# mapbox/robosat

Hardware: AMD Instinct MI355X
Metric: 512x512 tiles/sec train+predict, 1/2/4/8 MI355X; mIoU vs CPU ref (higher is better)
Workload: dtype f32; 1 GPU; rs predict ResNet50-UNet, bs=16 3x512x512 fp32 per GPU, 2 classes (BASELINE configs[1]); parallelism=tiles sharded over 1 rank(s), no collective

## Files before the change

include/robosat_hip.h:

```cpp
#ifndef ROBOSAT_HIP_H
#define ROBOSAT_HIP_H

#include <stdint.h>

#ifdef __cplusplus
extern "C" {
#endif

#define RS_EINVAL (-22)

typedef void* rs_stream_t;

typedef uint16_t rs_bf16;
#define RS_F32 0
#define RS_BF16 1

int rs_abi_version(void);

typedef struct rs_conv_desc {
  int32_t N;
  int32_t Hs, Ws;
  int32_t C1, C2;
  int32_t ups;
  int32_t kh, kw, stride, pad;
  int32_t Ho, Wo;
  int32_t Cout;
  int32_t relu;
  int32_t stem;
} rs_conv_desc;

int rs_conv2d_fwd(const rs_conv_desc* d, const float* src1, const float* src2, const float* weight,
                  const float* scale, const float* shift, const float* residual, const float* relu_mask, float* out,
                  rs_stream_t stream);

int rs_conv2d_tile(const rs_conv_desc* d);
const char* rs_conv2d_tile_name(int tile);

int rs_pack_stem_weight(const float* w_krsc, float* packed, int Cout, int kh, int kw, int Cin, rs_stream_t stream);


int rs_nchw_to_nhwc4(const float* x, float* y, int N, int C, int H, int W, rs_stream_t stream);

int rs_maxpool2d_fwd(const float* x, float* y, uint8_t* argmax, int N, int H, int W, int C, int k, int stride, int pad,
                     int Ho, int Wo, rs_stream_t stream);

int rs_bn_fold(const float* gamma, const float* beta, const float* mean, const float* var, float eps, float* scale,
               float* shift, int C, rs_stream_t stream);

int rs_final_conv1x1(const float* x, const float* w, const float* bias, float* out, int N, int H, int W, int Cin,
                     int C, int softmax, rs_stream_t stream);



long rs_conv2d_wgrad_workspace_bytes(const rs_conv_desc* d);
int rs_conv2d_wgrad_form(const rs_conv_desc* d);
int rs_conv2d_wgrad(const rs_conv_desc* d, const float* dy, const float* src1, const float* src2, float* dw,
                    void* workspace, rs_stream_t stream);
int rs_unpack_stem_weight(const float* packed, float* w_krsc, int Cout, int kh, int kw, int Cin, rs_stream_t stream);

int rs_pack_dgrad_weight(const float* w_krsc, float* out, int Cout, int kh, int kw, int Cin, rs_stream_t stream);

long rs_bn_workspace_bytes(long M, int C);
int rs_bn_train_stats(const float* y, long M, int C, float eps, float momentum, const float* gamma, const float* beta,
                      float* mean, float* invstd, float* scale, float* shift, float* running_mean, float* running_var,
                      long long* num_batches_tracked, void* workspace, rs_stream_t stream);
int rs_bn_apply(const float* y, const float* scale, const float* shift, const float* residual, float* out, long M, int C,
                int relu, rs_stream_t stream);
int rs_bn_bwd(const float* dz, const float* zmask, const float* y, const float* mean, const float* invstd,
              const float* gamma, float* dy, float* dmasked, float* dgamma, float* dbeta, long M, int C, void* workspace,
              rs_stream_t stream);

// ... 232 lines not shown
```

robosat_amd/_lib.py:

```python

import ctypes
import os
from ctypes import POINTER, c_char_p, c_float, c_int, c_int32, c_long, c_void_p

import torch

_HERE = os.path.dirname(os.path.abspath(__file__))
LIB_PATH = os.environ.get("ROBOSAT_HIP_LIB") or os.path.join(_HERE, "librobosat_hip.so")

RS_EINVAL = -22
ABI_VERSION = 24
RS_F32, RS_BF16 = 0, 1
RS_TTA_IN_U8, RS_TTA_IN_F32 = 0, 1
RS_TTA_PROBS, RS_TTA_QUANTIZE, RS_TTA_ARGMAX = 0, 1, 2


class ConvDesc(ctypes.Structure):

    _fields_ = [
        ("N", c_int32), ("Hs", c_int32), ("Ws", c_int32), ("C1", c_int32), ("C2", c_int32), ("ups", c_int32),
        ("kh", c_int32), ("kw", c_int32), ("stride", c_int32), ("pad", c_int32), ("Ho", c_int32), ("Wo", c_int32),
        ("Cout", c_int32), ("relu", c_int32), ("stem", c_int32),
    ]


P = c_void_p

SIGNATURES = {
    "rs_abi_version": (c_int, []),
    "rs_conv2d_fwd": (c_int, [POINTER(ConvDesc), P, P, P, P, P, P, P, P, P]),
    "rs_conv2d_tile": (c_int, [POINTER(ConvDesc)]),
    "rs_conv2d_tile_name": (c_char_p, [c_int]),
    "rs_pack_stem_weight": (c_int, [P, P, c_int, c_int, c_int, c_int, P]),
    "rs_nchw_to_nhwc4": (c_int, [P, P, c_int, c_int, c_int, c_int, P]),
    "rs_maxpool2d_fwd": (c_int, [P, P, P, c_int, c_int, c_int, c_int, c_int, c_int, c_int, c_int, c_int, P]),
    "rs_bn_fold": (c_int, [P, P, P, P, c_float, P, P, c_int, P]),
    "rs_final_conv1x1": (c_int, [P, P, P, P, c_int, c_int, c_int, c_int, c_int, c_int, P]),
    "rs_conv2d_wgrad_workspace_bytes": (c_long, [POINTER(ConvDesc)]),
    "rs_conv2d_wgrad": (c_int, [POINTER(ConvDesc), P, P, P, P, P, P]),
    "rs_unpack_stem_weight": (c_int, [P, P, c_int, c_int, c_int, c_int, P]),
    "rs_pack_dgrad_weight": (c_int, [P, P, c_int, c_int, c_int, c_int, P]),
    "rs_bn_workspace_bytes": (c_long, [c_long, c_int]),
    "rs_bn_train_stats": (c_int, [P, c_long, c_int, c_float, c_float, P, P, P, P, P, P, P, P, P, P, P]),
    "rs_bn_apply": (c_int, [P, P, P, P, P, c_long, c_int, c_int, P]),
    "rs_bn_bwd": (c_int, [P, P, P, P, P, P, P, P, P, P, c_long, c_int, P, P]),
    "rs_maxpool2d_bwd": (c_int, [P, P, P, c_int, c_int, c_int, c_int, c_int, c_int, c_int, c_int, c_int, c_int, P]),
    "rs_upsample2x_bwd": (c_int, [P, P, P, P, P, c_int, c_int, c_int, c_int, c_int, c_int, P]),
    "rs_final_conv1x1_bwd_workspace_bytes": (c_long, [c_int, c_int]),
    "rs_final_conv1x1_bwd": (c_int, [P, P, P, P, P, P, c_int, c_int, c_int, c_int, c_int, c_int, P, P]),
    "rs_nll_loss_workspace_bytes": (c_long, []),
    "rs_nll_loss_fwd": (c_int, [P, P, P, P, P, c_int, c_int, c_int, c_int, c_int, c_float, P, P]),
    "rs_nll_loss_bwd": (c_int, [P, P, P, P, P, P, c_int, c_int, c_int, c_int, c_int, c_float, P]),
    "rs_miou_loss_workspace_bytes": (c_long, [c_int, c_int]),
    "rs_miou_loss_fwd": (c_int, [P, P, P, P, P, c_int, c_int, c_int, c_int, P, P]),
    "rs_miou_loss_bwd": (c_int, [P, P, P, P, P, P, c_int, c_int, c_int, c_int, P]),
    "rs_lovasz_workspace_bytes": (c_long, [c_int, c_int, c_int, c_int]),
    "rs_lovasz_fwd": (c_int, [P, P, P, P, c_int, c_int, c_int, c_int, P, P]),
    "rs_scale_by_scalar": (c_int, [P, P, P, c_long, P]),
    "rs_lovasz_softmax_workspace_bytes": (c_long, [c_int, c_int, c_int, c_int, c_int]),
    "rs_lovasz_softmax_fwd": (c_int, [P, P, P, P, P, c_int, c_int, c_int, c_int, c_int, c_int, P, P]),
    "rs_confusion_counts": (c_int, [P, P, P, c_int, c_int, c_int, c_int, P]),
    "rs_conv2d_fwd_bf16": (c_int, [POINTER(ConvDesc), P, P, P, P, P, P, P, P, P]),
    "rs_conv2d_tile_bf16": (c_int, [POINTER(ConvDesc)]),
    "rs_conv2d_config": (c_int, [POINTER(ConvDesc), c_int, c_int, POINTER(c_int), POINTER(c_int)]),
    "rs_conv2d_set_tuning": (c_int, [c_int, c_int]),
    "rs_set_knob": (c_int, [c_char_p, c_int]),
# ... 131 lines not shown
```

robosat_amd/autograd.py:

```python

import torch

from . import ops


_SIDE = {}


def _side_stream(device):

    if torch.device(device).type != "cuda":
        return None
    if not ops.switch("ROBOSAT_WGRAD_STREAM"):
        return torch.cuda.current_stream(device)
    s = _SIDE.get(device)
    if s is None:
        s = torch.cuda.Stream(device=device)
        _SIDE[device] = s
    return s


class GradArena:

    TRACE = None
# ... 135 lines not shown
    ready.record(main)
    side.wait_event(ready)
    with torch.cuda.stream(side):
        packed = []
        for blk in (net.center, net.dec0, net.dec1, net.dec2, net.dec3, net.dec4):
            conv = blk.block.block
            packed += [conv.phase(dt), conv.dgrad_phase(dt)]
            if dt == torch.float32 and getattr(conv, "_phase_wino", None) is not None:
                packed.append(conv.phase_wino())
            if dt == torch.float32 and getattr(conv, "_dgrad_phase_wino", None) is not None:
                packed.append(conv.dgrad_phase_wino())
    done = torch.cuda.Event()
    done.record(side)
    for w in packed:
        w.record_stream(main)
    return done


def _forward(net, x, tape, backward=False):
    from .unet import _bump_generation

    _bump_generation()
    decoder_weights_ready = _prefetch_decoder_weights(net, net.compute_dtype, x.device)
    r = net.resnet
    t = tape.t
    dt = net.compute_dtype
    if dt == torch.bfloat16:
        net.prep_bf16_weights()
    elif backward:
        net.prep_f32_weights()
    x4 = ops.nchw_to_nhwc4(x, dt)
    t["x4"] = x4
    if dt == torch.bfloat16:
        y0 = ops.stem_conv_bf16(x4, ops.pack_stem_weight(r.conv1.krsc(), dt))
    else:
        y0 = ops.conv2d(x4, ops.pack_stem_weight(r.conv1.krsc()), stride=2, pad=3, stem=7, bands=net.in_channels)
    z0, st0 = _bn_train(r.bn1, y0)
    p0, am0 = ops.maxpool2d(z0, 3, 2, 1, want_argmax=True)
    t.update(y0=y0, st0=st0, z0=z0, am0=am0)

    h = p0
    enc = []
    for layer in net._blocks():
        for blk in layer:
            rec = {"blk": blk, "h": h}
            y1, z1, rec["st1"], rec["b1"] = _conv_bn(blk.bn1, h, blk.conv1.krsc(dt))
            y2, z2, rec["st2"], rec["b2"] = _conv_bn(blk.bn2, z1, blk.conv2.krsc(dt), stride=blk.stride, pad=1, conv=blk.conv2)
            if blk.downsample is not None:
                yd, idt, rec["std"], _ = _conv_bn(blk.downsample[1], h, blk.downsample[0].krsc(dt), stride=blk.stride, relu=False)
                rec["yd"] = yd
            else:
                idt = h
            y3, z3, rec["st3"], rec["b3"] = _conv_bn(blk.bn3, z2, blk.conv3.krsc(dt), residual=idt, relu=True)
            rec.update(y1=y1, z1=z1, y2=y2, z2=z2, y3=y3, z3=z3)
            tape.blocks.append(rec)
            h = z3
        enc.append(h)
    enc1, enc2, enc3, enc4 = enc

    def up(block, skip, prev=None):
        from .unet import decoder_block

        return decoder_block(block.block.block, skip, prev, dt)

    pooled, amc = ops.maxpool2d(enc4, 2, 2, 0, want_argmax=True)
    if decoder_weights_ready is not None:
        torch.cuda.current_stream(x.device).wait_event(decoder_weights_ready)
    center = up(net.center, pooled)
    dec0 = up(net.dec0, enc4, center)
# ... 198 lines not shown
```

robosat_amd/csrc/common.h:

```cpp
#pragma once
#include <hip/hip_runtime.h>
#include <stdint.h>

#include "../../include/robosat_hip.h"

typedef float f32x4 __attribute__((ext_vector_type(4)));
typedef float f32x16 __attribute__((ext_vector_type(16)));
typedef __bf16 bf16_t;
typedef __bf16 bf16x4 __attribute__((ext_vector_type(4)));
typedef __bf16 bf16x8 __attribute__((ext_vector_type(8)));
typedef unsigned int u32x2 __attribute__((ext_vector_type(2)));
typedef unsigned int u32x4 __attribute__((ext_vector_type(4)));
typedef short s16x4 __attribute__((ext_vector_type(4)));
typedef short s16x8 __attribute__((ext_vector_type(8)));

__device__ __forceinline__ f32x4 rs_ld4(const float* p) { return *reinterpret_cast<const f32x4*>(p); }
__device__ __forceinline__ f32x4 rs_ld4(const bf16_t* p) {
  return __builtin_convertvector(*reinterpret_cast<const bf16x4*>(p), f32x4);
}
__device__ __forceinline__ void rs_st4(float* p, f32x4 v) { *reinterpret_cast<f32x4*>(p) = v; }
__device__ __forceinline__ void rs_st4(bf16_t* p, f32x4 v) {
  *reinterpret_cast<bf16x4*>(p) = __builtin_convertvector(v, bf16x4);
}
__device__ __forceinline__ float rs_ld1(const float* p) { return *p; }
// ... 130 lines not shown
struct rs_fastdiv {
  unsigned int mul;
  unsigned int shift;
  unsigned int div;
};

static inline rs_fastdiv rs_make_fastdiv(unsigned int d) {
  rs_fastdiv f;
  unsigned int s = 0;
  while ((1ull << s) < d) ++s;
  f.shift = s;
  f.mul = (unsigned int)((((1ull << s) - d) << 32) / d + 1);
  f.div = d;
  return f;
}

__host__ __device__ __forceinline__ unsigned int rs_div(unsigned int n, const rs_fastdiv f) {
#if defined(__HIP_DEVICE_COMPILE__)
  return (__umulhi(n, f.mul) + n) >> f.shift;
#else
  return (unsigned int)((((unsigned long long)n * f.mul) >> 32) + n) >> f.shift;
#endif
}

struct RsKnobs {
  int conv_tile = -1;
  int conv_rowb = 0;
  int conv_big = 1;
  int conv_min256 = 384;
  int conv_halo = 1;
  int conv_halo_min = 192;
  int conv_halo512 = -1;
  int conv_splitk = -1;
  int conv1x1_ew = -1;
  int conv1x1_np = 0;
  int conv1x1_ew_bf16 = 0;
  int halo_ko = 0;
  int wgrad_f32_phase = 1;
  int wgrad_f32_dma = -1;
  int wgrad_f32_blocks = 2048;
  int wgrad_f32_wino = 1;
  int wgrad_f32_wino_blocks = 1024;
  int wgrad_f32_wino33 = 1;
  int wgrad_f32_wino33_blocks = 256;
  int wgrad_blocks = 96;
  int wgrad_blocks_phase = 1536;
  int wgrad_phase4 = 1;
  int wgrad_blocks_phase4 = 256;
  int wgrad_ring = 3;
  int lovasz_xcd = 1;
  int wino_wide = 1;
};
__attribute__((visibility("hidden"))) RsKnobs& rs_knobs();

__attribute__((visibility("hidden"))) int rs_wgrad_thin_plan(const rs_conv_desc* d, int* blocks, int* slices);
__attribute__((visibility("hidden"))) int rs_wgrad_thin_launch(const rs_conv_desc* d, const void* dy, const void* src,
                                                               float* partial, void* stream);

__attribute__((visibility("hidden"))) int rs_conv_thin_bf16_launch(int mode, const void* src, const void* wgt, const void* mask,
                                                                   void* out, int N, int Hs, int Ws, int relu, void* stream);

__attribute__((visibility("hidden"))) long rs_reduce_scratch_floats(long n, int splits);
__attribute__((visibility("hidden"))) int rs_reduce_splits(const float* ws, float* out, long n, int splits, float* scratch,
                                                           void* stream);

__attribute__((visibility("hidden"))) int rs_conv_dma_f32(const rs_conv_desc* d, const float* src1, const float* src2,
// ... 5 lines not shown
```

robosat_amd/csrc/knobs.hip:

```cpp
#include <stdio.h>
#include <stdlib.h>
#include <string.h>

#include "common.h"

namespace {

struct Entry {
  const char* name;
  const char* env;
  int RsKnobs::*field;
  int lo, hi;
};

bool in_range(const Entry& e, int v) {
  if (v < e.lo || v > e.hi) return false;
  if (e.field == &RsKnobs::conv_rowb) return v == 0 || v == 64 || v == 128;
  return true;
}

const Entry kEntries[] = {
    {"conv_tile", "RS_CONV_TILE", &RsKnobs::conv_tile, -1, 9},
    {"conv_rowb", "RS_CONV_ROWB", &RsKnobs::conv_rowb, 0, 128},
    {"conv_big", "RS_CONV_BIG", &RsKnobs::conv_big, 0, 1},
    {"conv_min256", "RS_CONV_MIN256", &RsKnobs::conv_min256, 0, 1048576},
    {"conv_halo", "RS_CONV_HALO", &RsKnobs::conv_halo, 0, 1},
    {"conv_halo_min", "RS_CONV_HALO_MIN", &RsKnobs::conv_halo_min, 0, 1048576},
    {"conv_halo512", "RS_CONV_HALO512", &RsKnobs::conv_halo512, -1, 1},
    {"conv_splitk", "RS_CONV_SPLITK", &RsKnobs::conv_splitk, -1, 16},
    {"conv1x1_ew", "RS_CONV1X1_EW", &RsKnobs::conv1x1_ew, -1, 1},
    {"conv1x1_np", "RS_CONV1X1_NP", &RsKnobs::conv1x1_np, -1, 1},
    {"conv1x1_ew_bf16", "RS_CONV1X1_EW_BF16", &RsKnobs::conv1x1_ew_bf16, 0, 1},
    {"halo_ko", "RS_HALO_KO", &RsKnobs::halo_ko, 0, 4},
    {"wgrad_f32_phase", "RS_WGRAD_F32_PHASE", &RsKnobs::wgrad_f32_phase, 0, 1},
    {"wgrad_f32_dma", "RS_WGRAD_F32_DMA", &RsKnobs::wgrad_f32_dma, -1, 1},
    {"wgrad_f32_blocks", "RS_WGRAD_F32_BLOCKS", &RsKnobs::wgrad_f32_blocks, 1, 1048576},
    {"wgrad_f32_wino", "RS_WGRAD_F32_WINO", &RsKnobs::wgrad_f32_wino, 0, 1},
    {"wgrad_f32_wino_blocks", "RS_WGRAD_F32_WINO_BLOCKS", &RsKnobs::wgrad_f32_wino_blocks, 1, 1048576},
    {"wgrad_f32_wino33", "RS_WGRAD_F32_WINO33", &RsKnobs::wgrad_f32_wino33, 0, 1},
    {"wgrad_f32_wino33_blocks", "RS_WGRAD_F32_WINO33_BLOCKS", &RsKnobs::wgrad_f32_wino33_blocks, 1, 1048576},
    {"wgrad_blocks", "RS_WGRAD_BLOCKS", &RsKnobs::wgrad_blocks, 1, 1048576},
    {"wgrad_blocks_phase", "RS_WGRAD_BLOCKS_PHASE", &RsKnobs::wgrad_blocks_phase, 1, 1048576},
    {"wgrad_phase4", "RS_WGRAD_PHASE4", &RsKnobs::wgrad_phase4, 0, 1},
    {"wgrad_blocks_phase4", "RS_WGRAD_BLOCKS_PHASE4", &RsKnobs::wgrad_blocks_phase4, 1, 1048576},
    {"wgrad_ring", "RS_WGRAD_RING", &RsKnobs::wgrad_ring, 2, 7},
    {"lovasz_xcd", "RS_LOVASZ_XCD", &RsKnobs::lovasz_xcd, 0, 1},
    {"wino_wide", "ROBOSAT_WINO_WIDE", &RsKnobs::wino_wide, 0, 1},
};

}

RsKnobs& rs_knobs() {
  static RsKnobs k = [] {
    RsKnobs v;
    for (const Entry& e : kEntries)
      if (const char* s = getenv(e.env)) {
        const int x = atoi(s);
        if (in_range(e, x)) v.*(e.field) = x;
        else fprintf(stderr, "robosat_hip: %s=%s is outside [%d, %d]: ignored, the rule stays\n", e.env, s, e.lo, e.hi);
      }
    return v;
  }();
// ... 24 lines not shown
```

robosat_amd/csrc/stem_f32.hip:

```cpp
#include "lds_dma.h"

namespace {

struct StemArgs {
  const float* x;
  const float* w;
  const float* scale;
  const float* shift;
  float* out;
  int N, H, W, Ho, Wo, relu;
  int tpr;
  int ntile;
#ifdef RS_STEM_TRACE
  long long* trace;
#endif
};

constexpr int SBM = 128, SBN = 64;
constexpr int SCOLS = 2 * SBM + 6;
constexpr int XI = 132;
constexpr int LDO = SBN + 4;

template <int CIN>
struct Geom {
  static constexpr int PS = CIN == 3 ? 3 : 5;
  static constexpr int ROWF = 2 * XI * PS;
  static constexpr int STRIPF = 7 * ROWF;
  static constexpr int PAIR = 7 * CIN;
  static constexpr int NPAIR = 3 * PAIR;
  static constexpr int NEO = 3 * CIN;
  static constexpr int NSTEP = NPAIR + NEO + CIN;
  static constexpr int WF = NSTEP * 2 * SBN;
  static constexpr int STAGEF = SBM * LDO;
  static constexpr int REGION = STRIPF > STAGEF ? STRIPF : STAGEF;
  static constexpr int ZEROF = SBM * PS + 8;
  static constexpr int LDSF = WF + REGION + ZEROF;
};

struct Tap {
  int r, s, c;
};
template <int CIN>
__host__ __device__ constexpr Tap stem_tap(int t, int h) {
  using G = Geom<CIN>;
  if (t < G::NPAIR) return Tap{2 * (t / G::PAIR) + h, (t % G::PAIR) / CIN, t % CIN};
  const int u = t - G::NPAIR;
  return Tap{6, 2 * (u / CIN) + h, u % CIN};
}
template <int CIN>
__host__ __device__ constexpr int stem_imm(int t) {
  using G = Geom<CIN>;
  const Tap k = stem_tap<CIN>(t, 0);
  return ((k.r * 2 + (k.s & 1)) * XI + (k.s >> 1)) * G::PS + k.c;
}

template <int CIN>
__global__ __launch_bounds__(256, CIN == 3 ? 2 : 1) void stem_conv_f32(const StemArgs p) {
  using G = Geom<CIN>;
  constexpr int PS = G::PS;
  constexpr int NPF = (7 * SCOLS + 255) / 256;
  static_assert(G::LDSF * 4 <= (CIN == 3 ? 80 : 160) * 1024, "LDS");

  __shared__ __attribute__((aligned(16))) float lds[G::LDSF];
  float* const wl = lds;
  float* const strip = lds + G::WF;
  float* const zline = lds + G::WF + G::REGION;

  const int tid = threadIdx.x;
  const int lane = tid & 63;
  const int wave = tid >> 6;
  const int wm = wave >> 1, wn = wave & 1;
  const int li = lane & 31, lh = lane >> 5;

#ifdef RS_STEM_TRACE
  if (tid == 0) p.trace[((long)blockIdx.x * 64 + 63) * 8 + 0] = (long long)__builtin_amdgcn_s_memtime();
#endif
  const int t0 = (int)((long)blockIdx.x * p.ntile / gridDim.x);
  const int t1 = (int)((long)(blockIdx.x + 1) * p.ntile / gridDim.x);
  if (t0 >= t1) return;

  {
    constexpr int NW4 = SBN * 7 * 8 / 256;
    f32x4 wv[NW4];
#pragma unroll
    for (int k = 0; k < NW4; ++k) wv[k] = *reinterpret_cast<const f32x4*>(p.w + (tid + 256 * k) * 4);
#pragma unroll
    for (int k = 0; k < NW4; ++k) {
      const int e = tid + 256 * k;
      const int s_ = e & 7, r = (e >> 3) % 7, co = e / 56;
      int t, h;
      if (r < 6) {
        t = (r >> 1) * G::PAIR + s_ * CIN, h = r & 1;
        if (s_ == 7) continue;
      } else if (s_ < 6) {
        t = G::NPAIR + (s_ >> 1) * CIN, h = s_ & 1;
      } else {
        t = G::NPAIR + G::NEO, h = s_ & 1;
      }
#pragma unroll
      for (int c = 0; c < CIN; ++c) wl[((t + c) * 2 + h) * SBN + co] = wv[k][c];
    }
  }
  for (int e = tid; e < G::ZEROF; e += 256) zline[e] = 0.f;

  f32x4 pf[NPF];
  int pdst[NPF];
  int prow[NPF], pcol[NPF], prel[NPF];
#pragma unroll
  for (int q = 0; q < NPF; ++q) {
    const int e = tid + 256 * q;
    const int r = e / SCOLS, j = e - r * SCOLS;
    const bool in = e < 7 * SCOLS;
    pdst[q] = in ? ((r * 2 + (j & 1)) * XI + (j >> 1)) * PS : -1;
    prow[q] = in ? r : -(1 << 24);
    pcol[q] = j;
    prel[q] = (r * p.W + j) * 16;
  }
  const long img = (long)p.H * p.W * 4;
  int cn, coy, ctx;
  {
    const int rowt = t0 / p.tpr;
    ctx = t0 - rowt * p.tpr;
    cn = rowt / p.Ho;
    coy = rowt - cn * p.Ho;
  }
  auto fetch = [&](int n, int oy, int tx, bool live) __attribute__((always_inline)) {
    const __amdgpu_buffer_rsrc_t rs = rs_dma_rsrc<0x7FFFFFF0u>(p.x + n * img, live ? img * 4 : 0);
    const int iy0 = 2 * oy - 3, ix0 = 2 * tx * SBM - 3;
    const int base = (iy0 * p.W + ix0) * 16;
#pragma unroll
    for (int q = 0; q < NPF; ++q) {
      const bool ok = (unsigned)(iy0 + prow[q]) < (unsigned)p.H && (unsigned)(ix0 + pcol[q]) < (unsigned)p.W;
      pf[q] = __builtin_bit_cast(f32x4, __builtin_amdgcn_raw_buffer_load_b128(rs, ok ? base + prel[q] : -1, 0, 0));
    }
  };
  auto put = [&]() __attribute__((always_inline)) {
#pragma unroll
    for (int q = 0; q < NPF; ++q) {
      if (pdst[q] >= 0) {
        float* d = strip + pdst[q];
        d[0] = pf[q][0];
        d[1] = pf[q][1];
        d[2] = pf[q][2];
        if (CIN == 4) d[3] = pf[q][3];
      }
    }
  };

  const int apix = (wm * 64 + li) * PS;
  const float* const A1 = strip + apix + lh * G::ROWF;
  const float* const A2 = strip + apix + lh * (XI * PS);
  constexpr int IMM6 = ((6 * 2 + 0) * XI + 3) * PS;
  const float* const A3 = lh ? zline + apix - IMM6 : strip + apix;
  const float* const B = wl + lh * SBN + wn * 32 + li;

  const int ecol = (tid & 15) * 4, erow = tid >> 4;
  f32x4 sc = {1.f, 1.f, 1.f, 1.f}, sh = {0.f, 0.f, 0.f, 0.f};
  if (p.scale) sc = *reinterpret_cast<const f32x4*>(p.scale + ecol);
  if (p.shift) sh = *reinterpret_cast<const f32x4*>(p.shift + ecol);

#ifdef RS_STEM_TRACE
#define STAMP(k) do { if (tid == 0) p.trace[((long)blockIdx.x * 64 + (tile - t0)) * 8 + (k)] = (long long)__builtin_amdgcn_s_memtime(); } while (0)
#else
#define STAMP(k)
#endif
#ifdef RS_STEM_TRACE
  if (tid == 0) p.trace[((long)blockIdx.x * 64 + 63) * 8 + 1] = (long long)__builtin_amdgcn_s_memtime();
#endif
  fetch(cn, coy, ctx, true);
  put();
  for (int tile = t0; tile < t1; ++tile) {
    STAMP(0);
    __syncthreads();
    STAMP(1);
    int nn = cn, noy = coy, ntx = ctx + 1;
    if (ntx == p.tpr) {
      ntx = 0;
      if (++noy == p.Ho) noy = 0, ++nn;
    }
    fetch(nn, noy, ntx, tile + 1 < t1);
    STAMP(2);

    f32x16 acc0, acc1;
#pragma unroll
    for (int r = 0; r < 16; ++r) acc0[r] = 0.f, acc1[r] = 0.f;
    constexpr int DEPTH = 3;
    float fb[DEPTH], fa0[DEPTH], fa1[DEPTH];
    auto frag = [&](int t) __attribute__((always_inline)) {
      const float* A = t < G::NPAIR ? A1 : (t < G::NPAIR + G::NEO ? A2 : A3);
      const int imm = stem_imm<CIN>(t);
      fb[t % DEPTH] = B[t * 2 * SBN];
      fa0[t % DEPTH] = A[imm];
      fa1[t % DEPTH] = A[imm + 32 * PS];
    };
#pragma unroll
    for (int t = 0; t < DEPTH; ++t) frag(t);
#pragma unroll
    for (int t = 0; t < G::NSTEP; ++t) {
      const float b = fb[t % DEPTH], a0 = fa0[t % DEPTH], a1 = fa1[t % DEPTH];
      __builtin_amdgcn_sched_barrier(0);
      acc0 = __builtin_amdgcn_mfma_f32_32x32x2f32(b, a0, acc0, 0, 0, 0);
      if (t + DEPTH < G::NSTEP) frag(t + DEPTH);
      acc1 = __builtin_amdgcn_mfma_f32_32x32x2f32(b, a1, acc1, 0, 0, 0);
      __builtin_amdgcn_sched_barrier(0);
    }
    STAMP(3);
    __syncthreads();
    STAMP(4);

    {
      const int prow = wm * 64 + li;
      const int ccol = wn * 32 + 4 * lh;
#pragma unroll
      for (int g = 0; g < 4; ++g) {
        *reinterpret_cast<f32x4*>(&strip[prow * LDO + ccol + 8 * g]) = f32x4{acc0[4 * g], acc0[4 * g + 1], acc0[4 * g + 2], acc0[4 * g + 3]};
        *reinterpret_cast<f32x4*>(&strip[(prow + 32) * LDO + ccol + 8 * g]) = f32x4{acc1[4 * g], acc1[4 * g + 1], acc1[4 * g + 2], acc1[4 * g + 3]};
      }
    }
    __syncthreads();
    f32x4 ov[SBM / 16];
#pragma unroll
    for (int i = 0; i < SBM / 16; ++i) ov[i] = *reinterpret_cast<const f32x4*>(&strip[(erow + 16 * i) * LDO + ecol]);
    __syncthreads();
    STAMP(5);
    put();
    STAMP(6);
    {
      const int ox0 = ctx * SBM;
      const int live = p.Wo - ox0 < SBM ? p.Wo - ox0 : SBM;
      float* const orow = p.out + (((long)cn * p.Ho + coy) * p.Wo + ox0) * SBN + ecol;
#pragma unroll
      for (int i = 0; i < SBM / 16; ++i) {
        const int row = erow + 16 * i;
        f32x4 v = ov[i];
#pragma unroll
        for (int e = 0; e < 4; ++e) v[e] = v[e] * sc[e] + sh[e];
        if (p.relu) {
#pragma unroll
          for (int e = 0; e < 4; ++e) v[e] = fmaxf(v[e], 0.f);
        }
        if (row < live) *reinterpret_cast<f32x4*>(orow + (long)row * SBN) = v;
      }
    }
    STAMP(7);
    cn = nn, coy = noy, ctx = ntx;
  }
#ifdef RS_STEM_TRACE
  if (tid == 0) p.trace[((long)blockIdx.x * 64 + 63) * 8 + 2] = (long long)__builtin_amdgcn_s_memtime();
#endif
}

}

__attribute__((visibility("hidden"))) int rs_stem_f32_launch(const rs_conv_desc* d, int bands, const float* x, const float* w,
                                                             const float* scale, const float* shift, float* out, void* stream) {
  if (d->kh != 7 || d->kw != 7 || d->stride != 2 || d->pad != 3 || d->Cout != SBN || d->C1 != 4) return RS_EINVAL;
  if (d->Ho != (d->Hs + 1) / 2 || d->Wo != (d->Ws + 1) / 2) return RS_EINVAL;
  if ((long)d->Hs * d->Ws * 16 >= (1L << 31)) return RS_EINVAL;
  StemArgs a;
  a.x = x, a.w = w, a.scale = scale, a.shift = shift, a.out = out;
  a.N = d->N, a.H = d->Hs, a.W = d->Ws, a.Ho = d->Ho, a.Wo = d->Wo, a.relu = d->relu;
  a.tpr = rs_cdiv(d->Wo, SBM);
  const long ntile = (long)d->N * d->Ho * a.tpr;
  if (ntile <= 0 || ntile >= (1L << 31)) return RS_EINVAL;
  a.ntile = (int)ntile;
  const int cus = rs_cu_count();
  const long want = bands == 3 ? 2L * cus : cus;
  const int grid = (int)(ntile < want ? ntile : want);
  if (bands == 3)
    stem_conv_f32<3><<<grid, 256, 0, (hipStream_t)stream>>>(a);
  else
    stem_conv_f32<4><<<grid, 256, 0, (hipStream_t)stream>>>(a);
  return RS_LAUNCH_RESULT();
}

#ifdef RS_STEM_TRACE
extern "C" int rs_stem_f32_trace(int N, int H, int W, const float* x, const float* w, float* out, long long* trace, int grid) {
  StemArgs a;
  a.x = x, a.w = w, a.scale = nullptr, a.shift = nullptr, a.out = out;
  a.N = N, a.H = H, a.W = W, a.Ho = H / 2, a.Wo = W / 2, a.relu = 1;
  a.tpr = rs_cdiv(a.Wo, SBM);
  a.ntile = N * a.Ho * a.tpr;
  a.trace = trace;
  stem_conv_f32<3><<<grid, 256, 0, 0>>>(a);
  return RS_LAUNCH_RESULT();
}
#endif
```

robosat_amd/ops.py:

```python

import ctypes
import os

import torch

from . import _lib
from ._lib import RS_BF16, RS_F32, ConvDesc, check

BF16 = torch.bfloat16


def _dt(t):

    dtype = getattr(t, "dtype", t)
    if dtype == torch.float32:
        return RS_F32
    if dtype == torch.bfloat16:
        return RS_BF16
    raise TypeError("robosat_amd: activations are fp32 or bf16, got {}".format(dtype))


def _esize(t):

    return 2 if getattr(t, "dtype", t) == BF16 else 4
# ... 681 lines not shown

    def __init__(self, weights_krsc, want_dgrad=True, dtype=BF16):

        assert weights_krsc and all(w.dtype == torch.float32 and w.is_contiguous() and w.dim() == 4 for w in weights_krsc)
        assert dtype == BF16 or want_dgrad
        dev = weights_krsc[0].device
        self.dtype = dtype
        self.weights = list(weights_krsc)
        self.cast = [torch.empty(w.shape, device=dev, dtype=BF16) if dtype == BF16 else None for w in self.weights]
        self.dgrad = [torch.empty((w.shape[3], w.shape[1], w.shape[2], w.shape[0]), device=dev, dtype=dtype) if want_dgrad else None
                      for w in self.weights]
        items = (_WPrepItem * len(self.weights))()
        tiles = 0
        for i, w in enumerate(self.weights):
            cout, kh, kw, cin = w.shape
            items[i] = _WPrepItem(_dev(w, "w").value, _dev(self.cast[i], "cast", BF16).value if dtype == BF16 else None,
                                  _dev(self.dgrad[i], "dgrad", dtype).value if want_dgrad else None, cout, kh * kw, cin, tiles)
            tiles += kh * kw * ((cin + 31) // 32) * ((cout + 31) // 32)
        self.tiles = tiles
        self.table = torch.frombuffer(bytearray(bytes(items)), dtype=torch.uint8).to(dev)
        self.ptrs = tuple(w.data_ptr() for w in self.weights)

    def run(self):
        _call("rs_weight_prep_bf16" if self.dtype == BF16 else "rs_weight_prep_f32", _dev(self.table, "items", torch.uint8),
              len(self.weights), self.tiles, _stream())


def pack_stem_weight(w_krsc, dtype=torch.float32):

    cout, kh, kw, cin = w_krsc.shape
    out = torch.empty((cout, kh, 8, 4), device=w_krsc.device, dtype=dtype)
    _call("rs_pack_stem_weight_bf16" if dtype == BF16 else "rs_pack_stem_weight", _dev(w_krsc, "w"), _dev(out, "out", dtype), cout, kh, kw,
          cin, _stream())
    return out


def nchw_to_nhwc4(x, dtype=torch.float32):
    n, c, h, w = x.shape
    out = torch.empty((n, h, w, 4), device=x.device, dtype=dtype)
    _call("rs_nchw_to_nhwc4_bf16" if dtype == BF16 else "rs_nchw_to_nhwc4", _dev(x, "x"), _dev(out, "out", dtype), n, c, h, w, _stream())
    return out


def stem_conv_bf16(x4, w_packed, scale=None, shift=None, relu=False):

    n, h, w, _ = x4.shape
    out = torch.empty((n, h // 2, w // 2, 64), device=x4.device, dtype=BF16)
    ev = _start()
    _call("rs_stem_conv_fwd_bf16", _dev(x4, "x4", BF16), _dev(w_packed, "w", BF16), _dev(scale, "scale"), _dev(shift, "shift"),
          _dev(out, "out", BF16), n, h, w, int(relu), _stream())
    if ev:
        _stop(ev)
        flops = 2.0 * n * 64 * 3 * 49 * (h // 2) * (w // 2)
        _record(ev, "stem_conv_bf16", flops, (3, 64, 7, 2, 0, h // 2, w // 2), 2 * (x4.numel() + out.numel()))
    return out


def wgrad_kernel_name(d, form=None):

    lib = _lib.lib()
    if form is None:
        form = lib.rs_conv2d_wgrad_bf16_form(ctypes.byref(d))
    if form == 1:
        return "conv_wgrad_thin_bf16<{}{}>".format(min(d.C1, 128), ",ups" if d.ups else "")
    t = lib.rs_conv2d_wgrad_bf16_tile(ctypes.byref(d))
    if t <= 0:
# ... 711 lines not shown
```

robosat_amd/unet.py:

```python

import math
import os
import warnings

import torch
import torch.nn as nn

from . import ops

_RESNET50_FILE = "resnet50-19c8e357.pth"


class _Conv(nn.Module):

    def __init__(self, cin, cout, k, stride=1, padding=0, bias=False, init="default"):
        super().__init__()
        self.cin, self.cout, self.k, self.stride, self.padding = cin, cout, k, stride, padding
        w = torch.empty(cout, cin, k, k).contiguous(memory_format=torch.channels_last)
        fan_in, fan_out = cin * k * k, cout * k * k
        if init == "resnet":
            nn.init.normal_(w, 0.0, math.sqrt(2.0 / fan_out))
        else:
            nn.init.uniform_(w, -1.0 / math.sqrt(fan_in), 1.0 / math.sqrt(fan_in))
        self.weight = nn.Parameter(w)
# ... 17 lines not shown

    def dgrad_weight(self, dtype=torch.float32):

        c = getattr(self, "_dgrad" if dtype == torch.bfloat16 else "_dgrad_f32", None)
        if c is not None and c[0] == (self.weight.data_ptr(), self.weight._version, _GENERATION[0]):
            return c[1]
        return ops.pack_dgrad_weight(self.krsc(), dtype)

    def phase(self, dtype=torch.float32):

        key = (self.weight.data_ptr(), self.weight._version, _GENERATION[0], dtype)
        c = getattr(self, "_phase", None)
        if c is None or c[0] != key:
            c = (key, ops.pack_phase_weight(self.krsc(), dtype))
            self._phase = c
        return c[1]

    def phase_wino(self):

        key = (self.weight.data_ptr(), self.weight._version, _GENERATION[0])
        c = getattr(self, "_phase_wino", None)
        if c is None or c[0] != key:
            c = (key, ops.pack_wino_phase_weight(self.phase(torch.float32)))
            self._phase_wino = c
        return c[1]

    def wino33(self):

        key = (self.weight.data_ptr(), self.weight._version, _GENERATION[0])
        c = getattr(self, "_wino33", None)
        if c is None or c[0] != key:
            c = (key, ops.pack_wino33_weight(self.krsc()))
            self._wino33 = c
        return c[1]

    def dgrad_wino33(self):

        key = (self.weight.data_ptr(), self.weight._version, _GENERATION[0])
        c = getattr(self, "_dgrad_wino33", None)
        if c is None or c[0] != key:
            c = (key, ops.pack_wino33_weight(self.dgrad_weight(torch.float32)))
            self._dgrad_wino33 = c
        return c[1]

    def dgrad_s2_phase(self, dtype=torch.float32, wino=False):

        key = (self.weight.data_ptr(), self.weight._version, _GENERATION[0], dtype, wino)
        c = getattr(self, "_dgrad_s2_phase", None)
        if c is None or c[0] != key:
            pack = ops.pack_s2_dgrad_phase_weight(self.krsc(), dtype)
            c = (key, ops.pack_wino_phase_weight(pack) if wino else pack)
            self._dgrad_s2_phase = c
        return c[1]

    def dgrad_phase(self, dtype=torch.float32):

        key = (self.weight.data_ptr(), self.weight._version, _GENERATION[0], dtype)
        c = getattr(self, "_dgrad_phase", None)
        if c is None or c[0] != key:
            c = (key, ops.pack_dgrad_phase_weight(self.krsc(), dtype))
            self._dgrad_phase = c
        return c[1]

    def dgrad_phase_wino(self):

        key = (self.weight.data_ptr(), self.weight._version, _GENERATION[0])
# ... 345 lines not shown
        assert images_u8.dtype == torch.uint8 and images_u8.dim() == 4 and images_u8.size(3) == self.in_channels
        assert images_u8.size(1) % 32 == 0 and images_u8.size(2) % 32 == 0, "image resolution has to be divisible by 32 for resnet"
        if not images_u8.is_cuda:
            raise RuntimeError("robosat_amd.UNet runs on the MI355X only (got a {} tensor); there is no CPU fallback".format(images_u8.device))
        mean, std = list(mean)[:self.in_channels], list(std)[:self.in_channels]
        if tta != "none":
            op_list = ops.tta_ops(tta, images_u8.size(1), images_u8.size(2))

            def run(u8):
                x4 = ops.tta_fan_out_u8(u8, mean, std, op_list, self.compute_dtype)
                return ops.tta_merge(self._forward_eval(None, softmax=True, x4=x4), op_list, "argmax")
        else:
            op_list = [0]

            def run(u8):
                x4 = ops.u8_to_nhwc4_norm(u8, mean, std)
                if self.compute_dtype == torch.bfloat16:
                    x4 = x4.to(torch.bfloat16)
                return self._forward_eval(None, softmax=False, x4=x4, argmax=True)

        images_u8 = images_u8.contiguous()
        if self._want_graph(images_u8, len(op_list)):
            return self._graph_replay(("classes", tuple(mean), tuple(std), tta), run, images_u8)
        return run(images_u8)

    def _forward_eval(self, x, softmax, x4=None, quantize_overlap=None, argmax=False):
        r = self.resnet
        dt = self.compute_dtype
        if x4 is None:
            if not x.is_cuda:
                raise RuntimeError("robosat_amd.UNet runs on the MI355X only (got a {} tensor); there is no CPU fallback".format(x.device))
            assert x.size(1) == self.in_channels
            x = x.detach().float().contiguous()
            x4 = ops.nchw_to_nhwc4(x, dt)
        h = x4
        sc, sh = r.bn1.folded()
        if dt == torch.bfloat16:
            h = ops.stem_conv_bf16(h, ops.pack_stem_weight(r.conv1.krsc(), dt), scale=sc, shift=sh, relu=True)
        else:
            h = ops.conv2d(h, ops.pack_stem_weight(r.conv1.krsc()), stride=2, pad=3, scale=sc, shift=sh, relu=True, stem=7,
                           bands=self.in_channels)
        h = ops.maxpool2d(h, 3, 2, 1)

        enc = []
        for layer in self._blocks():
            blocks = list(layer)
            ahead = None
            for bi, blk in enumerate(blocks):
                if ahead is None:
                    sc, sh = blk.bn1.folded()
                    o = ops.conv2d(h, blk.conv1.krsc(dt), scale=sc, shift=sh, relu=True)
                else:
                    o, ahead = ahead, None
                sc, sh = blk.bn2.folded()
                o = conv3x3_eval(blk.conv2, o, dt, scale=sc, shift=sh)
                if blk.downsample is not None:
                    sc, sh = blk.downsample[1].folded()
                    dw = blk.downsample[0].krsc(dt)
                    if blk.stride == 1 and ops.conv1x1_wave_ok(h, dw):
                        idt = ops.conv1x1_wave(h, dw, sc, sh)
                    else:
                        idt = ops.conv2d(h, dw, stride=blk.stride, scale=sc, shift=sh)
                else:
                    idt = h
                sc, sh = blk.bn3.folded()
                nxt = blocks[bi + 1] if bi + 1 < len(blocks) else None
                if (nxt is not None and nxt.conv1.k == 1 and nxt.conv1.stride == 1 and dt == torch.float32
                        and ops.bottleneck_tail_ok(o, blk.conv3.krsc(dt), nxt.conv1.krsc(dt))):
                    sc1, sh1 = nxt.bn1.folded()
                    h, ahead = ops.bottleneck_tail(o, blk.conv3.krsc(dt), sc, sh, idt, nxt.conv1.krsc(dt), sc1, sh1)
                else:
                    h = ops.conv2d(o, blk.conv3.krsc(dt), scale=sc, shift=sh, residual=idt, relu=True)
            enc.append(h)
        enc1, enc2, enc3, enc4 = enc

# ... 21 lines not shown
```

Baseline: 1656 tiles/s.

## Fuse stem maxpool into f32 stem conv and read NCHW input directly

Adds a pooled variant of the f32 7x7 stem conv kernel that applies BN/ReLU and the 3x3 stride-2 maxpool in-kernel, carrying row and column state across tiles so the full-resolution stem activation is never written. An NCHW-input form lets the eval path skip the separate nchw_to_nhwc4 conversion kernel. The packed stem weight is also cached per module instead of repacked every forward. The cost is recomputing seed rows at block boundaries, extra register pressure, and a more complex kernel.

```diff
diff --git a/include/robosat_hip.h b/include/robosat_hip.h
--- a/include/robosat_hip.h
+++ b/include/robosat_hip.h
@@ -37,6 +37,10 @@
 const char* rs_conv2d_tile_name(int tile);
 
 int rs_pack_stem_weight(const float* w_krsc, float* packed, int Cout, int kh, int kw, int Cin, rs_stream_t stream);
+
+int rs_stem_pool_plan(const rs_conv_desc* d, int* blocks, int* seed_rows);
+int rs_stem_conv_fwd_f32(const rs_conv_desc* d, int flags, const float* x, const float* w_packed, const float* scale,
+                         const float* shift, float* out, rs_stream_t stream);
 
 
 int rs_nchw_to_nhwc4(const float* x, float* y, int N, int C, int H, int W, rs_stream_t stream);
diff --git a/robosat_amd/_lib.py b/robosat_amd/_lib.py
--- a/robosat_amd/_lib.py
+++ b/robosat_amd/_lib.py
@@ -32,6 +32,8 @@
     "rs_conv2d_tile": (c_int, [POINTER(ConvDesc)]),
     "rs_conv2d_tile_name": (c_char_p, [c_int]),
     "rs_pack_stem_weight": (c_int, [P, P, c_int, c_int, c_int, c_int, P]),
+    "rs_stem_pool_plan": (c_int, [POINTER(ConvDesc), POINTER(c_int), POINTER(c_int)]),
+    "rs_stem_conv_fwd_f32": (c_int, [POINTER(ConvDesc), c_int, P, P, P, P, P, P]),
     "rs_nchw_to_nhwc4": (c_int, [P, P, c_int, c_int, c_int, c_int, P]),
     "rs_maxpool2d_fwd": (c_int, [P, P, P, c_int, c_int, c_int, c_int, c_int, c_int, c_int, c_int, c_int, P]),
     "rs_bn_fold": (c_int, [P, P, P, P, c_float, P, P, c_int, P]),
diff --git a/robosat_amd/autograd.py b/robosat_amd/autograd.py
--- a/robosat_amd/autograd.py
+++ b/robosat_amd/autograd.py
@@ -191,9 +191,9 @@
     x4 = ops.nchw_to_nhwc4(x, dt)
     t["x4"] = x4
     if dt == torch.bfloat16:
-        y0 = ops.stem_conv_bf16(x4, ops.pack_stem_weight(r.conv1.krsc(), dt))
-    else:
-        y0 = ops.conv2d(x4, ops.pack_stem_weight(r.conv1.krsc()), stride=2, pad=3, stem=7, bands=net.in_channels)
+        y0 = ops.stem_conv_bf16(x4, r.conv1.stem_pack(dt))
+    else:
+        y0 = ops.conv2d(x4, r.conv1.stem_pack(), stride=2, pad=3, stem=7, bands=net.in_channels)
     z0, st0 = _bn_train(r.bn1, y0)
     p0, am0 = ops.maxpool2d(z0, 3, 2, 1, want_argmax=True)
     t.update(y0=y0, st0=st0, z0=z0, am0=am0)
diff --git a/robosat_amd/csrc/common.h b/robosat_amd/csrc/common.h
--- a/robosat_amd/csrc/common.h
+++ b/robosat_amd/csrc/common.h
@@ -186,6 +186,7 @@
   int conv_halo_min = 192;
   int conv_halo512 = -1;
   int conv_splitk = -1;
+  int stem_pool = -1;
   int conv1x1_ew = -1;
   int conv1x1_np = 0;
   int conv1x1_ew_bf16 = 0;
diff --git a/robosat_amd/csrc/knobs.hip b/robosat_amd/csrc/knobs.hip
--- a/robosat_amd/csrc/knobs.hip
+++ b/robosat_amd/csrc/knobs.hip
@@ -28,6 +28,7 @@
     {"conv_halo_min", "RS_CONV_HALO_MIN", &RsKnobs::conv_halo_min, 0, 1048576},
     {"conv_halo512", "RS_CONV_HALO512", &RsKnobs::conv_halo512, -1, 1},
     {"conv_splitk", "RS_CONV_SPLITK", &RsKnobs::conv_splitk, -1, 16},
+    {"stem_pool", "RS_STEM_POOL", &RsKnobs::stem_pool, -1, 1048576},
     {"conv1x1_ew", "RS_CONV1X1_EW", &RsKnobs::conv1x1_ew, -1, 1},
     {"conv1x1_np", "RS_CONV1X1_NP", &RsKnobs::conv1x1_np, -1, 1},
     {"conv1x1_ew_bf16", "RS_CONV1X1_EW_BF16", &RsKnobs::conv1x1_ew_bf16, 0, 1},
diff --git a/robosat_amd/csrc/stem_f32.hip b/robosat_amd/csrc/stem_f32.hip
--- a/robosat_amd/csrc/stem_f32.hip
+++ b/robosat_amd/csrc/stem_f32.hip
@@ -20,6 +20,7 @@
 constexpr int SCOLS = 2 * SBM + 6;
 constexpr int XI = 132;
 constexpr int LDO = SBN + 4;
+constexpr int NQ4 = (SCOLS + 2) / 4;
 
 template <int CIN>
 struct Geom {
@@ -54,17 +55,20 @@
   return ((k.r * 2 + (k.s & 1)) * XI + (k.s >> 1)) * G::PS + k.c;
 }
 
-template <int CIN>
+template <int CIN, bool POOL = false, bool NCHW = false>
 __global__ __launch_bounds__(256, CIN == 3 ? 2 : 1) void stem_conv_f32(const StemArgs p) {
   using G = Geom<CIN>;
   constexpr int PS = G::PS;
-  constexpr int NPF = (7 * SCOLS + 255) / 256;
-  static_assert(G::LDSF * 4 <= (CIN == 3 ? 80 : 160) * 1024, "LDS");
-
-  __shared__ __attribute__((aligned(16))) float lds[G::LDSF];
+  constexpr int NPF = NCHW ? (CIN * 7 * NQ4 + 255) / 256 : (7 * SCOLS + 255) / 256;
+  constexpr int LDSF = G::LDSF + (POOL ? SBN : 0);
+  static_assert(LDSF * 4 <= (CIN == 3 ? 80 : 160) * 1024, "LDS");
+
+  __shared__ __attribute__((aligned(16))) float lds[LDSF];
   float* const wl = lds;
   float* const strip = lds + G::WF;
   float* const zline = lds + G::WF + G::REGION;
+  float* const carry = lds + G::LDSF;
+  static_assert(G::LDSF % 4 == 0, "the carried column is read and written 16 bytes at a time");
 
   const int tid = threadIdx.x;
   const int lane = tid & 63;
@@ -75,9 +79,22 @@
 #ifdef RS_STEM_TRACE
   if (tid == 0) p.trace[((long)blockIdx.x * 64 + 63) * 8 + 0] = (long long)__builtin_amdgcn_s_memtime();
 #endif
-  const int t0 = (int)((long)blockIdx.x * p.ntile / gridDim.x);
-  const int t1 = (int)((long)(blockIdx.x + 1) * p.ntile / gridDim.x);
-  if (t0 >= t1) return;
+  int t0, t1;
+  int tlive = 0;
+  if constexpr (POOL) {
+    const int np = p.N * (p.Ho >> 1);
+    const int g0 = (int)((long)blockIdx.x * np / gridDim.x);
+    const int g1 = (int)((long)(blockIdx.x + 1) * np / gridDim.x);
+    if (g0 >= g1) return;
+    const int seed = (2 * g0) % p.Ho != 0;
+    tlive = 2 * g0 * p.tpr;
+    t0 = (2 * g0 - seed) * p.tpr;
+    t1 = 2 * g1 * p.tpr;
+  } else {
+    t0 = (int)((long)blockIdx.x * p.ntile / gridDim.x);
+    t1 = (int)((long)(blockIdx.x + 1) * p.ntile / gridDim.x);
+    if (t0 >= t1) return;
+  }
 
   {
     constexpr int NW4 = SBN * 7 * 8 / 256;
@@ -109,14 +126,23 @@
 #pragma unroll
   for (int q = 0; q < NPF; ++q) {
     const int e = tid + 256 * q;
-    const int r = e / SCOLS, j = e - r * SCOLS;
-    const bool in = e < 7 * SCOLS;
-    pdst[q] = in ? ((r * 2 + (j & 1)) * XI + (j >> 1)) * PS : -1;
-    prow[q] = in ? r : -(1 << 24);
-    pcol[q] = j;
-    prel[q] = (r * p.W + j) * 16;
-  }
-  const long img = (long)p.H * p.W * 4;
+    if constexpr (NCHW) {
+      const int m = e % NQ4, r = (e / NQ4) % 7, c = e / (7 * NQ4);
+      const bool in = e < CIN * 7 * NQ4;
+      pdst[q] = in ? (r * 2 * XI + 2 * m) * PS + c : -1;
+      prow[q] = in ? r : -(1 << 24);
+      pcol[q] = 4 * m;
+      prel[q] = ((c * p.H + r) * p.W + 4 * m) * 4;
+    } else {
+      const int r = e / SCOLS, j = e - r * SCOLS;
+      const bool in = e < 7 * SCOLS;
+      pdst[q] = in ? ((r * 2 + (j & 1)) * XI + (j >> 1)) * PS : -1;
+      prow[q] = in ? r : -(1 << 24);
+      pcol[q] = j;
+      prel[q] = (r * p.W + j) * 16;
+    }
+  }
+  const long img = (long)p.H * p.W * (NCHW ? CIN : 4);
   int cn, coy, ctx;
   {
     const int rowt = t0 / p.tpr;
@@ -126,8 +152,8 @@
   }
   auto fetch = [&](int n, int oy, int tx, bool live) __attribute__((always_inline)) {
     const __amdgpu_buffer_rsrc_t rs = rs_dma_rsrc<0x7FFFFFF0u>(p.x + n * img, live ? img * 4 : 0);
-    const int iy0 = 2 * oy - 3, ix0 = 2 * tx * SBM - 3;
-    const int base = (iy0 * p.W + ix0) * 16;
+    const int iy0 = 2 * oy - 3, ix0 = 2 * tx * SBM - (NCHW ? 4 : 3);
+    const int base = (iy0 * p.W + ix0) * (NCHW ? 4 : 16);
 #pragma unroll
     for (int q = 0; q < NPF; ++q) {
       const bool ok = (unsigned)(iy0 + prow[q]) < (unsigned)p.H && (unsigned)(ix0 + pcol[q]) < (unsigned)p.W;
@@ -139,10 +165,17 @@
     for (int q = 0; q < NPF; ++q) {
       if (pdst[q] >= 0) {
         float* d = strip + pdst[q];
-        d[0] = pf[q][0];
-        d[1] = pf[q][1];
-        d[2] = pf[q][2];
-        if (CIN == 4) d[3] = pf[q][3];
+        if constexpr (NCHW) {
+          d[(XI - 1) * PS] = pf[q][0];
+          d[0] = pf[q][1];
+          d[XI * PS] = pf[q][2];
+          d[PS] = pf[q][3];
+        } else {
+          d[0] = pf[q][0];
+          d[1] = pf[q][1];
+          d[2] = pf[q][2];
+          if (CIN == 4) d[3] = pf[q][3];
+        }
       }
     }
   };
@@ -167,6 +200,11 @@
 #ifdef RS_STEM_TRACE
   if (tid == 0) p.trace[((long)blockIdx.x * 64 + 63) * 8 + 1] = (long long)__builtin_amdgcn_s_memtime();
 #endif
+  f32x4 B0[4], B1[4];
+  if constexpr (POOL) {
+#pragma unroll
+    for (int i = 0; i < 4; ++i) B0[i] = f32x4{0.f, 0.f, 0.f, 0.f}, B1[i] = f32x4{0.f, 0.f, 0.f, 0.f};
+  }
   fetch(cn, coy, ctx, true);
   put();
   for (int tile = t0; tile < t1; ++tile) {
@@ -218,28 +256,90 @@
       }
     }
     __syncthreads();
-    f32x4 ov[SBM / 16];
-#pragma unroll
-    for (int i = 0; i < SBM / 16; ++i) ov[i] = *reinterpret_cast<const f32x4*>(&strip[(erow + 16 * i) * LDO + ecol]);
-    __syncthreads();
-    STAMP(5);
-    put();
-    STAMP(6);
-    {
-      const int ox0 = ctx * SBM;
-      const int live = p.Wo - ox0 < SBM ? p.Wo - ox0 : SBM;
-      float* const orow = p.out + (((long)cn * p.Ho + coy) * p.Wo + ox0) * SBN + ecol;
-#pragma unroll
-      for (int i = 0; i < SBM / 16; ++i) {
-        const int row = erow + 16 * i;
-        f32x4 v = ov[i];
-#pragma unroll
-        for (int e = 0; e < 4; ++e) v[e] = v[e] * sc[e] + sh[e];
-        if (p.relu) {
-#pragma unroll
-          for (int e = 0; e < 4; ++e) v[e] = fmaxf(v[e], 0.f);
+    if constexpr (POOL) {
+      f32x4 hv[4][3];
+#pragma unroll
+      for (int i = 0; i < 4; ++i) {
+        const int j = erow + 16 * i;
+        const float* const left = (i == 0 && erow == 0) ? carry + ecol : &strip[(2 * j - 1) * LDO + ecol];
+        hv[i][0] = *reinterpret_cast<const f32x4*>(left);
+        hv[i][1] = *reinterpret_cast<const f32x4*>(&strip[(2 * j) * LDO + ecol]);
+        hv[i][2] = *reinterpret_cast<const f32x4*>(&strip[(2 * j + 1) * LDO + ecol]);
+      }
+      __syncthreads();
+      if (erow == 15) *reinterpret_cast<f32x4*>(carry + ecol) = hv[3][2];
+      STAMP(5);
+      put();
+      STAMP(6);
+      f32x4 h[4];
+#pragma unroll
+      for (int i = 0; i < 4; ++i) {
+#pragma unroll
+        for (int k = 0; k < 3; ++k) {
+#pragma unroll
+          for (int e = 0; e < 4; ++e) hv[i][k][e] = hv[i][k][e] * sc[e] + sh[e];
+          if (p.relu) {
+#pragma unroll
+            for (int e = 0; e < 4; ++e) hv[i][k][e] = fmaxf(hv[i][k][e], 0.f);
+          }
         }
-        if (row < live) *reinterpret_cast<f32x4*>(orow + (long)row * SBN) = v;
+        const bool has_left = i > 0 || erow > 0 || ctx > 0;
+#pragma unroll
+        for (int e = 0; e < 4; ++e) {
+          const float m = fmaxf(hv[i][1][e], hv[i][2][e]);
+          h[i][e] = has_left ? fmaxf(m, hv[i][0][e]) : m;
+        }
+      }
+      const int wp = p.Wo >> 1, px0 = ctx * (SBM / 2);
+      const int livep = wp - px0 < SBM / 2 ? wp - px0 : SBM / 2;
+      float* const orow = p.out + (((long)cn * (p.Ho >> 1) + (coy >> 1)) * wp + px0) * SBN + ecol;
+      const bool odd = coy & 1, store = tile >= tlive;
+      auto vpool = [&](f32x4(&Bx)[4]) __attribute__((always_inline)) {
+#pragma unroll
+        for (int i = 0; i < 4; ++i) {
+          if (odd) {
+            f32x4 o;
+#pragma unroll
+            for (int e = 0; e < 4; ++e) o[e] = fmaxf(Bx[i][e], h[i][e]);
+            if (store && erow + 16 * i < livep) *reinterpret_cast<f32x4*>(orow + (long)(erow + 16 * i) * SBN) = o;
+            Bx[i] = h[i];
+          } else if (coy == 0) {
+            Bx[i] = h[i];
+          } else {
+#pragma unroll
+            for (int e = 0; e < 4; ++e) Bx[i][e] = fmaxf(Bx[i][e], h[i][e]);
+          }
+        }
+      };
+      if (ctx == 0)
+        vpool(B0);
+      else
+        vpool(B1);
+      rs_lds_writes_done();
+    } else {
+      f32x4 ov[SBM / 16];
+#pragma unroll
+      for (int i = 0; i < SBM / 16; ++i) ov[i] = *reinterpret_cast<const f32x4*>(&strip[(erow + 16 * i) * LDO + ecol]);
+      __syncthreads();
+      STAMP(5);
+      put();
+      STAMP(6);
+      {
+        const int ox0 = ctx * SBM;
+        const int live = p.Wo - ox0 < SBM ? p.Wo - ox0 : SBM;
+        float* const orow = p.out + (((long)cn * p.Ho + coy) * p.Wo + ox0) * SBN + ecol;
+#pragma unroll
+        for (int i = 0; i < SBM / 16; ++i) {
+          const int row = erow + 16 * i;
+          f32x4 v = ov[i];
+#pragma unroll
+          for (int e = 0; e < 4; ++e) v[e] = v[e] * sc[e] + sh[e];
+          if (p.relu) {
+#pragma unroll
+            for (int e = 0; e < 4; ++e) v[e] = fmaxf(v[e], 0.f);
+          }
+          if (row < live) *reinterpret_cast<f32x4*>(orow + (long)row * SBN) = v;
+        }
       }
     }
     STAMP(7);
@@ -250,13 +350,38 @@
 #endif
 }
 
-}
-
-__attribute__((visibility("hidden"))) int rs_stem_f32_launch(const rs_conv_desc* d, int bands, const float* x, const float* w,
-                                                             const float* scale, const float* shift, float* out, void* stream) {
-  if (d->kh != 7 || d->kw != 7 || d->stride != 2 || d->pad != 3 || d->Cout != SBN || d->C1 != 4) return RS_EINVAL;
-  if (d->Ho != (d->Hs + 1) / 2 || d->Wo != (d->Ws + 1) / 2) return RS_EINVAL;
-  if ((long)d->Hs * d->Ws * 16 >= (1L << 31)) return RS_EINVAL;
+bool stem_geometry(const rs_conv_desc* d) {
+  if (!d || d->N <= 0 || d->Hs <= 0 || d->Ws <= 0) return false;
+  if (d->kh != 7 || d->kw != 7 || d->stride != 2 || d->pad != 3 || d->Cout != SBN || d->C1 != 4) return false;
+  if (d->Ho != (d->Hs + 1) / 2 || d->Wo != (d->Ws + 1) / 2) return false;
+  return (long)d->Hs * d->Ws * 16 < (1L << 31);
+}
+
+bool pool_plan(const rs_conv_desc* d, int bands, int* blocks, int* seeds) {
+  const int knob = rs_knobs().stem_pool;
+  if (!stem_geometry(d) || knob == 0 || (d->Ho & 1) || (d->Wo & 1) || d->Wo > 2 * SBM) return false;
+  const long np = (long)d->N * (d->Ho / 2);
+  const long want = knob > 0 ? knob : (bands == 3 ? 2L : 1L) * rs_cu_count();
+  const int grid = (int)(np < want ? np : want);
+  int ns = 0;
+  for (int b = 0; b < grid; ++b) ns += (2 * (b * np / grid)) % d->Ho != 0;
+  if (blocks) *blocks = grid;
+  if (seeds) *seeds = ns;
+  return true;
+}
+
+template <bool POOL, bool NCHW>
+void launch_form(int bands, int grid, const StemArgs& a, hipStream_t s) {
+  if (bands == 3)
+    stem_conv_f32<3, POOL, NCHW><<<grid, 256, 0, s>>>(a);
+  else
+    stem_conv_f32<4, POOL, NCHW><<<grid, 256, 0, s>>>(a);
+}
+
+int stem_launch(const rs_conv_desc* d, int bands, bool pool, bool nchw, const float* x, const float* w, const float* scale,
+                const float* shift, float* out, void* stream) {
+  if (!stem_geometry(d)) return RS_EINVAL;
+  if (nchw && ((d->Ws & 3) || ((unsigned long)x & 15) || (long)d->Hs * d->Ws * 4 * bands >= (1L << 31))) return RS_EINVAL;
   StemArgs a;
   a.x = x, a.w = w, a.scale = scale, a.shift = shift, a.out = out;
   a.N = d->N, a.H = d->Hs, a.W = d->Ws, a.Ho = d->Ho, a.Wo = d->Wo, a.relu = d->relu;
@@ -264,14 +389,43 @@
   const long ntile = (long)d->N * d->Ho * a.tpr;
   if (ntile <= 0 || ntile >= (1L << 31)) return RS_EINVAL;
   a.ntile = (int)ntile;
-  const int cus = rs_cu_count();
-  const long want = bands == 3 ? 2L * cus : cus;
-  const int grid = (int)(ntile < want ? ntile : want);
-  if (bands == 3)
-    stem_conv_f32<3><<<grid, 256, 0, (hipStream_t)stream>>>(a);
+  int grid;
+  if (pool) {
+    if (!pool_plan(d, bands, &grid, nullptr)) return RS_EINVAL;
+  } else {
+    const long want = (bands == 3 ? 2L : 1L) * rs_cu_count();
+    grid = (int)(ntile < want ? ntile : want);
+  }
+  const hipStream_t s = (hipStream_t)stream;
+  if (pool && nchw)
+    launch_form<true, true>(bands, grid, a, s);
+  else if (pool)
+    launch_form<true, false>(bands, grid, a, s);
+  else if (nchw)
+    launch_form<false, true>(bands, grid, a, s);
+  else if (bands == 3)
+    stem_conv_f32<3><<<grid, 256, 0, s>>>(a);
   else
-    stem_conv_f32<4><<<grid, 256, 0, (hipStream_t)stream>>>(a);
+    stem_conv_f32<4><<<grid, 256, 0, s>>>(a);
   return RS_LAUNCH_RESULT();
+}
+
+}
+
+__attribute__((visibility("hidden"))) int rs_stem_f32_launch(const rs_conv_desc* d, int bands, const float* x, const float* w,
+                                                             const float* scale, const float* shift, float* out, void* stream) {
+  return stem_launch(d, bands, false, false, x, w, scale, shift, out, stream);
+}
+
+extern "C" int rs_stem_pool_plan(const rs_conv_desc* d, int* blocks, int* seed_rows) {
+  if (!d || !d->stem) return RS_EINVAL;
+  return pool_plan(d, d->stem == 3 ? 3 : 4, blocks, seed_rows) ? 1 : 0;
+}
+
+extern "C" int rs_stem_conv_fwd_f32(const rs_conv_desc* d, int flags, const float* x, const float* w, const float* scale,
+                                    const float* shift, float* out, rs_stream_t stream) {
+  if (!d || !d->stem || !x || !w || !out || (flags & ~3)) return RS_EINVAL;
+  return stem_launch(d, d->stem == 3 ? 3 : 4, flags & 1, flags & 2, x, w, scale, shift, out, stream);
 }
 
 #ifdef RS_STEM_TRACE
diff --git a/robosat_amd/ops.py b/robosat_amd/ops.py
--- a/robosat_amd/ops.py
+++ b/robosat_amd/ops.py
@@ -737,6 +737,51 @@
     out = torch.empty((cout, kh, 8, 4), device=w_krsc.device, dtype=dtype)
     _call("rs_pack_stem_weight_bf16" if dtype == BF16 else "rs_pack_stem_weight", _dev(w_krsc, "w"), _dev(out, "out", dtype), cout, kh, kw,
           cin, _stream())
+    return out
+
+
+def _stem_desc(n, h, w, relu, bands):
+    return ConvDesc(n, h, w, 4, 0, 0, 7, 7, 2, 3, (h + 1) // 2, (w + 1) // 2, 64, int(relu), 3 if bands <= 3 else 1)
+
+
+def stem_pool_plan(h, w, dtype=torch.float32, bands=3, n=1):
+
+    if dtype != torch.float32:
+        return None
+    blocks, seeds = ctypes.c_int(0), ctypes.c_int(0)
+    rc = _lib.lib().rs_stem_pool_plan(ctypes.byref(_stem_desc(n, h, w, False, bands)), ctypes.byref(blocks), ctypes.byref(seeds))
+    if rc < 0:
+        check(rc, "rs_stem_pool_plan")
+    return (blocks.value, seeds.value) if rc else None
+
+
+def stem_pool_ok(h, w, dtype=torch.float32, bands=3):
+
+    return stem_pool_plan(h, w, dtype, bands) is not None
+
+
+def stem_conv(x, w_packed, scale=None, shift=None, relu=False, bands=4, nchw=False, pool=False):
+
+    if nchw:
+        n, c, h, w = x.shape
+        if c != bands or bands not in (3, 4):
+            raise ValueError("stem_conv(nchw=True) reads 3 or 4 planes, one per band: got {} planes, bands = {}".format(c, bands))
+    else:
+        n, h, w, c = x.shape
+        assert c == 4
+    d = _stem_desc(n, h, w, relu, bands)
+    plan = stem_pool_plan(h, w, x.dtype, bands, n) if pool else None
+    if pool and plan is None:
+        raise ValueError("stem_conv(pool=True): no pooled form for {}x{} {} images (ops.stem_pool_ok)".format(h, w, x.dtype))
+    out = torch.empty((n, d.Ho // 2, d.Wo // 2, 64) if pool else (n, d.Ho, d.Wo, 64), device=x.device, dtype=torch.float32)
+    ev = _start()
+    _call("rs_stem_conv_fwd_f32", ctypes.byref(d), int(bool(pool)) | 2 * int(bool(nchw)), _dev(x, "x"), _dev(w_packed, "w"),
+          _dev(scale, "scale"), _dev(shift, "shift"), _dev(out, "out"), _stream())
+    if ev:
+        _stop(ev)
+        rows = d.N * d.Ho
+        _record(ev, conv_tile_name(d), conv_flops(d), _shape(d), 4 * (x.numel() + d.Cout * d.kh * d.kw * 4 + out.numel()),
+                conv_flops(d) * (rows + plan[1]) / rows if pool else None)
     return out
 
 
diff --git a/robosat_amd/unet.py b/robosat_amd/unet.py
--- a/robosat_amd/unet.py
+++ b/robosat_amd/unet.py
@@ -73,6 +73,15 @@
         if c is None or c[0] != key:
             c = (key, ops.pack_wino33_weight(self.krsc()))
             self._wino33 = c
+        return c[1]
+
+    def stem_pack(self, dtype=torch.float32):
+
+        key = (self.weight.data_ptr(), self.weight._version, _GENERATION[0], dtype)
+        c = getattr(self, "_stem_pack", None)
+        if c is None or c[0] != key:
+            c = (key, ops.pack_stem_weight(self.krsc(), dtype))
+            self._stem_pack = c
         return c[1]
 
     def dgrad_wino33(self):
@@ -484,15 +493,19 @@
                 raise RuntimeError("robosat_amd.UNet runs on the MI355X only (got a {} tensor); there is no CPU fallback".format(x.device))
             assert x.size(1) == self.in_channels
             x = x.detach().float().contiguous()
-            x4 = ops.nchw_to_nhwc4(x, dt)
-        h = x4
+            nchw = dt == torch.float32 and self.in_channels >= 3 and x.size(3) % 4 == 0
+            h = x if nchw else ops.nchw_to_nhwc4(x, dt)
+            hw = x.shape[2:]
+        else:
+            nchw, h, hw = False, x4, x4.shape[1:3]
         sc, sh = r.bn1.folded()
         if dt == torch.bfloat16:
-            h = ops.stem_conv_bf16(h, ops.pack_stem_weight(r.conv1.krsc(), dt), scale=sc, shift=sh, relu=True)
+            h = ops.maxpool2d(ops.stem_conv_bf16(h, r.conv1.stem_pack(dt), scale=sc, shift=sh, relu=True), 3, 2, 1)
         else:
-            h = ops.conv2d(h, ops.pack_stem_weight(r.conv1.krsc()), stride=2, pad=3, scale=sc, shift=sh, relu=True, stem=7,
-                           bands=self.in_channels)
-        h = ops.maxpool2d(h, 3, 2, 1)
+            pool = ops.stem_pool_ok(hw[0], hw[1], dt, self.in_channels)
+            h = ops.stem_conv(h, r.conv1.stem_pack(), scale=sc, shift=sh, relu=True, bands=self.in_channels, nchw=nchw, pool=pool)
+            if not pool:
+                h = ops.maxpool2d(h, 3, 2, 1)
 
         enc = []
         for layer in self._blocks():
```

After: 1670 tiles/s (median of 6 runs). Within noise of the previous version (+0.9%).
